# masa-ue/SVDD

Measured on AMD Instinct MI355X. Metric: decoded sequences/sec (whole node), L=200 M=10 128-step SVDD-MC, higher is better.
Workload: dtype f32; 1 GPU; DNA enhancer SVDD-MC, batch=256/GPU, L=200, M=10, 128 steps (BASELINE.json configs[1]); dilated-CNN backbone 3.3M params + ConvGRU value net; global_batch=256, rng=philox

## Files before the change

include/svdd_hip.h:

```cpp
#ifndef SVDD_HIP_H
#define SVDD_HIP_H

#include <stdint.h>

#ifdef __cplusplus
extern "C" {
#endif

#define SVDD_VOCAB 5
#define SVDD_MASK 4
#define SVDD_MAX_M 1024

enum {
  SVDD_OK = 0,
  SVDD_E_ARG = -1,
  SVDD_E_LAUNCH = -2,
  SVDD_E_NODEVICE = -3
};

enum {
  SVDD_LAYOUT_BLV = 0,
  SVDD_LAYOUT_BVL = 1
};

// ... 121 lines not shown

int svdd_transform_samples(const uint8_t* tok, int R, int L, int transposed, float* out,
                           void* stream);

int svdd_subs_logp(const float* logits, const uint8_t* x, int B, int L, int layout, float* logp,
                   void* stream);

int svdd_compact_flags(const int32_t* flags, int n, int32_t* live_idx, int32_t* slot, int32_t* count, void* stream);
int svdd_compact_by_key(const int32_t* key, int n, int32_t* live_idx, int32_t* slot, int32_t* count, int split, void* stream);
int svdd_gather_rows(const void* src, const int32_t* idx, const int32_t* count, int n, int row_bytes, void* dst, void* stream);
int svdd_advance_rows(const void* src, const int32_t* slot, const int32_t* sel, int B, int M, int row_bytes, void* dst,
                      void* stream);
int svdd_select_compact(const float* scores, const int32_t* slot, const float* parent_score, const uint8_t* cand, int B,
                        int L, int M, int mode, const svdd_rng_t* rng, uint8_t* x_next, float* soft, int32_t* idx,
                        float* sel_score, int32_t* changed, void* stream);

int svdd_tds_resample(const float* reward_num, const float* reward_den, double alpha,
                      const uint8_t* sample, const double* u, int B, int L,
                      uint8_t* x_next, int32_t* idx, double* work, void* stream);

int svdd_mt19937_uniform_f32(uint32_t* state, float* out, long long n, void* stream);

int svdd_gru_bidir_f32(const float* x, const float* wpack, const float* bpack, float* out, int n, int L,
                       const int32_t* count, void* stream);

int svdd_bb_layer_fwd_f32(const float* y, const float* bias, const float* f_prev, const float* tb, const float* gamma,
                          const float* beta, float eps, float* f_out, uint8_t* mask, float* hn, int64_t rows, int rows_per_seq,
                          int channels, void* stream);
int svdd_bb_layer_bwd_f32(const float* g_hn, const float* f_in, const float* tb, const float* gamma, float eps, const float* g_in,
                          const uint8_t* mask_prev, float* g_out, float* gt_out, int64_t rows, int rows_per_seq, int channels,
// ... 158 lines not shown
```

svdd_amd/_lib.py:

```python
import ctypes
import os
import subprocess

_HERE = os.path.dirname(os.path.abspath(__file__))
CSRC = os.path.join(_HERE, "csrc")
SO_PATH = os.environ.get("SVDD_HIP_LIB") or os.path.join(CSRC, "libsvdd_hip.so")
ABI_VERSION = 17

OK, E_ARG, E_LAUNCH, E_NODEVICE = 0, -1, -2, -3
LAYOUT_BLV, LAYOUT_BVL = 0, 1
RNG_REPLAY, RNG_PHILOX = 0, 1
SELECT_ARGMAX, SELECT_MULTINOMIAL = 0, 1
TARGET_MEAN, TARGET_LOGMEANEXP = 0, 1
EVOLVE_GLOBAL, EVOLVE_ROW = 0, 1
ATTR_GRADIENT, ATTR_TIMES_INPUT = 0, 1
PRECISIONS = {"f32": 0, "f16x3": 1, "bf16x3": 2, "f16": 3, "bf16": 4}
MAX_M = 1024
PATTERN_MAX_WIDTH = 32

OPT_FORCE_EXACT, OPT_MSPLIT, OPT_SELECT_ONE_ROW, OPT_BACKBONE_LP_VERSION, OPT_TRUNK_GEMM_VERSION = 0, 1, 2, 3, 4
OPT_CAND_ROW_STRIDE, OPT_TRUNK_PLANES_F32, OPT_BACKBONE_SPLIT, OPT_SELECT_BATCHES = 5, 6, 7, 8


class SvddRng(ctypes.Structure):
# ... 104 lines not shown
                         vp, vp, vp, vp, vp, vp, vp, vp, vp, vp, vp),
    "svdd_candidate_windows_tight": (vp, vp, i32, i32, i32, i32, vp, vp, vp),
    "svdd_kmer_counts": (vp, i32, i32, i32, vp, vp, vp),
    "svdd_pack_tokens": (vp, i32, i32, vp, vp, vp),
    "svdd_hamming_nn": (vp, vp, i32, i32, i32, i32, i32, i32, vp, vp, vp),
    "svdd_edit_nn": (vp, vp, i32, i32, i32, i32, i32, i32, i32, i32, vp, vp, vp),
    "svdd_within": (vp, vp, vp, vp, i32, i32, i32, i32, vp, vp, i32, vp),
    "svdd_greedy_pick": (vp, i32, vp, vp, i32, i32, i32, i32, vp, vp, vp, i32, vp, vp),
    "svdd_edit_within": (vp, vp, vp, i32, i32, i32, i32, i32, vp, vp, i32, vp),
    "svdd_edit_pairs": (vp, vp, vp, i32, i32, i32, i32, i32, i32, vp, vp),
    "svdd_motif_scan": (vp, i32, i32, vp, vp, vp, i32, i32, vp, vp, vp, vp, vp),
    "svdd_motif_reward": (vp, i32, i32, vp, vp, vp, vp, i32, i32, vp, vp, vp, vp, vp, f32, vp, vp, vp, vp),
    "svdd_candidate_parts": (vp, vp, i32, i32, i32, i32, i32, vp, vp, vp, vp, vp),
    "svdd_conv_tower_parts_f32": (vp, vp, vp, vp, vp, vp, i32, i32, i32, i32, i32, i32, vp, vp, vp),
    "svdd_backbone_incr4_f32": (vp, vp, vp, vp, vp, vp, i32, i32, i32, pi32, i32, vp, vp, vp, vp, i32, i32, vp, vp, i32, vp, i32, vp),
    "svdd_pattern_mutants": (vp, vp, vp, vp, vp, i32, i32, i32, i32, vp, vp, vp, vp),
    "svdd_pattern_fold": (vp, vp, vp, vp, i32, i32, i32, i32, i32, vp, vp, vp, vp, vp),
    "svdd_pattern_apply": (vp, vp, vp, vp, vp, vp, i32, i32, i32, i32, i32, vp, vp, vp, vp, vp, vp, vp, vp, vp, vp, vp, vp),
}
EXPORTS = tuple(SIGNATURES)


def build(force=False):
    import glob
    srcs = sorted(glob.glob(os.path.join(CSRC, "*.hip")) + glob.glob(os.path.join(CSRC, "*.h")) + [os.path.join(CSRC, "Makefile")])
    srcs.append(os.path.join(os.path.dirname(_HERE), "include", "svdd_hip.h"))
    if os.environ.get("SVDD_HIP_LIB"):
        return SO_PATH
    stale = not os.path.exists(SO_PATH) or os.path.getmtime(SO_PATH) < max(os.path.getmtime(f) for f in srcs)
    if force or stale:
# ... 123 lines not shown
```

svdd_amd/csrc/svdd_kernels.hip:

```cpp
#include <float.h>
#include <stdlib.h>
#include <string.h>

#include "svdd_host.h"

namespace {

constexpr int V = SVDD_VOCAB;
constexpr int MASK = SVDD_MASK;
constexpr float NEG_INF_F = -1000000.0f;
constexpr int WAVE = 64;

__device__ __forceinline__ float expf_cr(float x) { return (float)exp((double)x); }
__device__ __forceinline__ float logf_cr(float x) { return (float)log((double)x); }
__device__ __forceinline__ float expf_cr_small(float x) {
  const double d = (double)x;
  double p = 1.0 / 720.0;
  p = __builtin_fma(p, d, 1.0 / 120.0);
  p = __builtin_fma(p, d, 1.0 / 24.0);
  p = __builtin_fma(p, d, 1.0 / 6.0);
  p = __builtin_fma(p, d, 0.5);
  p = __builtin_fma(p, d, 1.0);
  p = __builtin_fma(p, d, 1.0);
  const long long low = __double_as_longlong(p) & 0x1FFFFFFFll;
// ... 1986 lines not shown
  const int b = blockIdx.x;
  const int sl = slot[(size_t)b * M + sel[b]];
  if (sl < 0) return;
  const uintptr_t al = (uintptr_t)row_bytes | reinterpret_cast<uintptr_t>(src) | reinterpret_cast<uintptr_t>(dst);
  if ((al & 15) == 0) {
    const uint4* s16 = reinterpret_cast<const uint4*>(src + (size_t)sl * row_bytes);
    uint4* d16 = reinterpret_cast<uint4*>(dst + (size_t)b * row_bytes);
    for (int i = threadIdx.x; i < (row_bytes >> 4); i += 256) d16[i] = s16[i];
  } else {
    const uint32_t* s4 = reinterpret_cast<const uint32_t*>(src + (size_t)sl * row_bytes);
    uint32_t* d4 = reinterpret_cast<uint32_t*>(dst + (size_t)b * row_bytes);
    for (int i = threadIdx.x; i < (row_bytes >> 2); i += 256) d4[i] = s4[i];
  }
}


constexpr int MT_N = 624, MT_M = 397, MT_GEN = MT_N - MT_M , MT_RING = 2048;

__device__ __forceinline__ uint32_t mt_tw(uint32_t a, uint32_t b) {
  const uint32_t y = (a & 0x80000000u) | (b & 0x7fffffffu);
  return (y >> 1) ^ ((b & 1u) ? 0x9908b0dfu : 0u);
}
__device__ __forceinline__ uint32_t mt_temper(uint32_t y) {
  y ^= (y >> 11);
  y ^= (y << 7) & 0x9d2c5680u;
  y ^= (y << 15) & 0xefc60000u;
  y ^= (y >> 18);
  return y;
}
__device__ __forceinline__ float mt_float(uint32_t x) { return (float)(mt_temper(x) & 0xFFFFFFu) * (1.0f / 16777216.0f); }
// ... 297 lines not shown

int svdd_gather_rows(const void* src, const int32_t* idx, const int32_t* count, int n, int row_bytes, void* dst, void* stream) {
  if (!src || !idx || !dst || n <= 0 || row_bytes <= 0) return SVDD_E_ARG;
  return svdd_launch(gather_rows_kernel, dim3((unsigned)((n + 3) / 4)), dim3(256), 0, stream, (const uint8_t*)src, idx, count, n,
                     row_bytes, (uint8_t*)dst);
}

int svdd_advance_rows(const void* src, const int32_t* slot, const int32_t* sel, int B, int M, int row_bytes, void* dst,
                      void* stream) {
  if (!src || !slot || !sel || !dst || B <= 0 || M <= 0 || row_bytes <= 0 || (row_bytes & 3)) return SVDD_E_ARG;
  if (((uintptr_t)src | (uintptr_t)dst) & 3) return SVDD_E_ARG;
  return svdd_launch(advance_rows_kernel, dim3((unsigned)B), dim3(256), 0, stream, (const uint8_t*)src, slot, sel, B, M, row_bytes,
                     (uint8_t*)dst);
}

static int launch_pos(void (*k)(PosArgs), const PosArgs& a, void* stream) {
  const int64_t N = (int64_t)a.R * a.L;
  return svdd_launch(k, dim3((unsigned)((N + 255) / 256)), dim3(256), 0, stream, a);
}

int svdd_x0hat(const float* logits, const uint8_t* xt, int R, int L, int layout, float* onehot_t, uint8_t* x0hat,
               void* stream) {
  if (!logits || !xt || (!onehot_t && !x0hat) || R <= 0 || L <= 0 || bad_layout(layout)) return SVDD_E_ARG;
  return launch_pos(x0hat_kernel, PosArgs{logits, xt, R, L, layout, onehot_t, x0hat, nullptr, 1}, stream);
}

int svdd_finalize(const float* logits, const uint8_t* x, int B, int L, int layout, int64_t* out_i64,
                  uint8_t* out_u8, void* stream) {
  if (!logits || !x || (!out_i64 && !out_u8) || B <= 0 || L <= 0 || bad_layout(layout)) return SVDD_E_ARG;
  return launch_pos(finalize_kernel, PosArgs{logits, x, B, L, layout, nullptr, out_u8, out_i64, 0}, stream);
// ... 291 lines not shown
```

svdd_amd/csrc/svdd_nets.hip:

```cpp
#include "svdd_host.h"
#include "svdd_device.h"

namespace {

constexpr int H = 64;
constexpr int HPAD = H + 4;

template <bool BOTH>
__global__ __launch_bounds__(BOTH ? 512 : 256) void gru_bidir_kernel(const float* __restrict__ x, const float* __restrict__ wpack,
                                                                     const float* __restrict__ bpack, float* __restrict__ out,
                                                                     int n_alloc, int L, int ts, const int* __restrict__ count) {
  __shared__ __attribute__((aligned(16))) float hbuf_all[BOTH ? 2 : 1][2][TS][HPAD];
  const int lane = threadIdx.x & 63;
  const int w = (threadIdx.x >> 6) & 3;
  const int dir = BOTH ? (int)(threadIdx.x >> 8) : (int)(blockIdx.x & 1);
  float (*hbuf)[TS][HPAD] = hbuf_all[BOTH ? dir : 0];
  const int j = lane & 15;
  const int g = lane >> 4;
  const int seq0 = (BOTH ? (int)blockIdx.x : (int)(blockIdx.x >> 1)) * ts;
  const int n = count ? __builtin_amdgcn_readfirstlane(*count) : n_alloc;
  if (seq0 >= n) return;

  float wr[96];
  {
// ... 1736 lines not shown
  for (int e = tid; e < tile_rows * 5; e += 512) {
    const int row = e / 5, v = e - 5 * row;
    const int q = SPT1 ? 0 : row % il, pos = SPT1 ? row : row / il;
    if (seq0 + q >= nvalid) continue;
    const float* hr = img + row * BB_AP;
    const float* wv = a.w2 + v * BB_C;
    float sm = a.w2[5 * BB_C + v];
#pragma unroll 8
    for (int k = 0; k < BB_C; ++k) sm += hr[k] * wv[k];
    const int64_t sq = (a.row_idx && a.out_scatter) ? (int64_t)a.row_idx[seq0 + q] : (int64_t)(seq0 + q);
    a.out[(sq * L + pos) * 5 + v] = sm;
  }
}
#undef BB_OWN

constexpr int SEG_SLOTS = 7;

struct BackboneSegArgs {
  const uint8_t* x;
  const float* table0;
  const float* tiles;
  const float* vec;
  float* planes;
  const int* items;
  int n, L, layer;
  const int* order;
  const int* order_count;
  int order_stride;
};

struct BackboneReach {
  int r[BB_MAXL];
// ... 158 lines not shown
        unsigned m = 0;
        if (rr < n)
          for (int e = 0; e < 8 && 8 * w8 + e < L; ++e) {
            const size_t at = (size_t)rr * L + 8 * w8 + e;
            const uint8_t a = x[at];
            if (keep) x_next[at] = a;
            m |= (unsigned)(a != x_cur[at]) << e;
          }
        chb[rl * 32 + w8] = (unsigned char)m;
      }
    }
    __syncthreads();
    const int r = r0 + tid;
    const u64 ch[4] = {chs[tid][0], chs[tid][1], chs[tid][2], chs[tid][3]};
    int* it = its[tid];
    int cnt = 0, nt = 0;
    if (tight) {
      int cend = -1, io = 0, il = 0;
#pragma unroll
      for (int q = 0; q < 4; ++q)
        for (u64 b = ch[q]; b; b &= b - 1) {
          const int p = 64 * q + __builtin_ctzll(b);
          const int lo = max(0, p - reach), hi = min(L - 1, p + reach);
          int o = lo > cend ? lo : cend + 1;
          for (; o <= hi; o += 16) {
            ++nt;
            if (il > 0 && il < max_item && o == io + 16 * il) { ++il; continue; }
            if (il > 0) { if (cnt < SEG_SLOTS) it[cnt] = io | il << 8; ++cnt; }
            io = o; il = 1;
          }
          cend = o - 1;
        }
      if (il > 0) { if (cnt < SEG_SLOTS) it[cnt] = io | il << 8; ++cnt; }
    }
    if (!tight || cnt > SEG_SLOTS) {
      int m = 0;
#pragma unroll
      for (int q = 0; q < 4; ++q)
        for (u64 b = ch[q]; b; b &= b - 1) {
          const int p = 64 * q + __builtin_ctzll(b);
          const int tlo = max(0, p - reach) >> 4, thi = min(L - 1, p + reach) >> 4;
          m |= ((2 << thi) - 1) & ~((1 << tlo) - 1);
        }
      cnt = 0; nt = __popc(m);
      for (int t = 0; t < TW_RT;) {
        if (!(m >> t & 1)) { ++t; continue; }
        int len = 1;
        while (len < max_item && t + len < TW_RT && (m >> (t + len) & 1)) ++len;
        it[cnt++] = (tight ? 16 * t : t) | len << 8;
        t += len;
      }
    }
    for (; cnt < SEG_SLOTS; ++cnt) it[cnt] = 0;
    tiles += nt;
#pragma unroll
    for (int s = 0; s < SEG_SLOTS; ++s) {
      item[s] = its[tid][s];
      if (r < n) itk[(size_t)r * SEG_SLOTS + s] = item[s];
#pragma unroll
      for (int c = 0; c < 4; ++c) cnt4[c] += (item[s] >> 8) == 4 - c;
    }
    __syncthreads();
  }
  if (stat) {
#pragma unroll
    for (int off = 32; off > 0; off >>= 1) tiles += __shfl_xor(tiles, off, 64);
    if (lane == 0 && tiles) atomicAdd(stat + (tight ? 0 : 1), (unsigned long long)tiles);
  }
// ... 909 lines not shown
static size_t seg_lds_bytes(int rows, bool pad) {
  size_t bytes = sizeof(float) * ((size_t)rows * BB_AP + 5 * (size_t)rows + rows + 8);
  if (pad && g_incr_residency > 0) {
    const size_t least = (CU_LDS_BYTES / (size_t)(g_incr_residency + 1) / 1024 + 1) * 1024;
    if (least > bytes) bytes = least;
  }
  return bytes;
}

enum IncrList { INCR_SLOT, INCR_ORDERED, INCR_TIGHT };

struct IncrCall {
  const uint8_t* x; const float *table0, *tiles, *vec, *w2; float* out; int n, L, nlayers; const int* dilations; int lead;
  float* planes; uint8_t* x_prev; int32_t* items; unsigned long long* stat; int first, max_item;
  int32_t *order, *order_count; int depth; uint8_t* x_prev2; int parity; void* stream;
};

typedef void (*BackboneSegKernel)(BackboneSegArgs);
static BackboneSegKernel backbone_seg_choice(IncrList list, int mi, bool dilation4) {
  if (dilation4) return mi == 4 ? backbone_seg_kernel<4, true, 4> : mi == 2 ? backbone_seg_kernel<2, true, 4> : backbone_seg_kernel<1, true, 4>;
  if (list == INCR_TIGHT) return backbone_seg_tight_kernel;
  if (list == INCR_SLOT) return mi == 4 ? backbone_seg_kernel<4> : backbone_seg_kernel<2>;
  return mi == 4 ? backbone_seg_kernel<4, true> : mi == 2 ? backbone_seg_kernel<2, true> : backbone_seg_kernel<1, true>;
}

static int backbone_incr(IncrList list, const IncrCall& c) {
  const bool ordered = list != INCR_SLOT, tight = list == INCR_TIGHT;
  const int n = c.n, L = c.L, mi = c.max_item, lead = c.lead, depth = c.depth;
  if (!c.x || !c.table0 || !c.tiles || !c.vec || !c.w2 || !c.out || !c.dilations || !c.planes || !c.x_prev || !c.items || n <= 0 ||
      L <= TW_ROWS / 2 || L > TW_ROWS || c.nlayers <= 0 || c.nlayers > BB_MAXL || lead < 2 || lead > c.nlayers || depth < lead ||
      depth > c.nlayers || !(mi == 2 || (mi == 4 && !tight) || (mi == 1 && list == INCR_ORDERED)) ||
      (ordered && (!c.order || !c.order_count || n > 65536)) ||
      (tight && (!c.x_prev2 || c.x_prev2 == c.x_prev || (c.parity != 0 && c.parity != 1))))
    return SVDD_E_ARG;
  for (int i = 0; i < depth; ++i) if (c.dilations[i] != (i < lead ? 1 : 4)) return SVDD_E_ARG;
  BackboneArgs a;
  if (!backbone_args(a, c.x, c.table0, c.tiles, c.vec, c.w2, c.out, n, L, 1, c.nlayers, c.dilations)) return SVDD_E_ARG;
  a.planes = c.planes; a.planes_P = depth;
  uint8_t* x_cur = c.parity ? c.x_prev2 : c.x_prev;
  uint8_t* x_next = c.parity ? c.x_prev : c.x_prev2;
  const SvddLds lds = svdd_lds_raised(backbone_lds_bytes(c.nlayers, 3));
  SvddSpan span(SVDD_SLOT_BACKBONE);
  if (c.first) {
    if (hipMemcpyAsync(x_cur, c.x, (size_t)n * L, hipMemcpyDeviceToDevice, (hipStream_t)c.stream) != hipSuccess) return SVDD_E_LAUNCH;
    return svdd_launch_timed(span.all(), backbone_kernel<true, false, 1>, dim3((unsigned)n), dim3(512), lds, c.stream, a, BackboneSave{});
  }
  const int slots = mi == 1 ? TW_RT : SEG_SLOTS;
  const BackboneReach reach = backbone_reach(c.dilations, depth, lead);
  int rc;
  if (tight) {
    rc = svdd_launch_timed(span.first(), backbone_list_kernel, dim3((unsigned)depth), dim3(256), 0, c.stream, c.x, (const uint8_t*)x_cur, x_next,
                           n, L, mi, c.items, c.order, c.order_count, c.stat, reach);
  } else {
    rc = svdd_launch_timed(span.first(), mi == 1 ? backbone_worklist_kernel<TW_RT> : backbone_worklist_kernel<SEG_SLOTS>,
                           dim3((unsigned)((n + 3) / 4)), dim3(256), 0, c.stream, c.x, c.x_prev, n, L, depth, mi, c.items, c.stat, reach);
    if (rc == SVDD_OK && ordered)
      rc = svdd_launch(mi == 1 ? backbone_order_kernel<TW_RT> : backbone_order_kernel<SEG_SLOTS>, dim3((unsigned)depth), dim3(256), 0, c.stream,
                       c.items, n, c.order, c.order_count);
  }
  if (rc != SVDD_OK) return SVDD_E_LAUNCH;
  BackboneSegArgs sa{c.x, c.table0, c.tiles, c.vec, c.planes, c.items, n, L, 0, nullptr, nullptr, 0};
  if (ordered) { sa.order = c.order; sa.order_count = c.order_count; sa.order_stride = n * slots; }
  const BackboneSegKernel seg[2] = {backbone_seg_choice(list, mi, false), backbone_seg_choice(list, mi, true)};
  const size_t slds[2] = {seg_lds_bytes(tight ? 16 * mi + 8 : 16 * (mi + 2), ordered), seg_lds_bytes(16 * (mi + 2), ordered)};
  svdd_raise_lds_limit(seg[0], slds[0]);
  if (depth > lead) svdd_raise_lds_limit(seg[1], slds[1]);
  const dim3 sgrid((unsigned)n * slots);
  for (int k = 1; k <= depth; ++k) {
    sa.layer = k;
    if (svdd_launch(seg[k > lead], sgrid, dim3(256), slds[k > lead], c.stream, sa) != SVDD_OK) return SVDD_E_LAUNCH;
  }
  return svdd_launch_timed(span.last(), backbone_kernel<true, false, 2>, dim3((unsigned)n), dim3(512), lds, c.stream, a, BackboneSave{});
}

extern "C" int svdd_backbone_incr_f32(const uint8_t* x, const float* table0, const float* tiles, const float* vec, const float* w2,
                                      float* out, int n, int L, int nlayers, const int* dilations, int lead, float* planes,
                                      uint8_t* x_prev, int32_t* items, unsigned long long* stat, int first, int max_item,
                                      void* stream) {
  return backbone_incr(INCR_SLOT, IncrCall{x, table0, tiles, vec, w2, out, n, L, nlayers, dilations, lead, planes, x_prev, items, stat, first,
                                           max_item, nullptr, nullptr, lead, nullptr, 0, stream});
}

extern "C" int svdd_backbone_incr2_f32(const uint8_t* x, const float* table0, const float* tiles, const float* vec, const float* w2,
                                       float* out, int n, int L, int nlayers, const int* dilations, int lead, float* planes,
                                       uint8_t* x_prev, int32_t* items, unsigned long long* stat, int first, int max_item,
// ... 5 lines not shown
extern "C" int svdd_backbone_incr3_f32(const uint8_t* x, const float* table0, const float* tiles, const float* vec, const float* w2,
                                       float* out, int n, int L, int nlayers, const int* dilations, int lead, float* planes,
                                       uint8_t* x_prev, int32_t* items, unsigned long long* stat, int first, int max_item,
                                       int32_t* order, int32_t* order_count, int depth, void* stream) {
  return backbone_incr(INCR_ORDERED, IncrCall{x, table0, tiles, vec, w2, out, n, L, nlayers, dilations, lead, planes, x_prev, items, stat, first,
                                              max_item, order, order_count, depth, nullptr, 0, stream});
}

extern "C" int svdd_backbone_incr4_f32(const uint8_t* x, const float* table0, const float* tiles, const float* vec, const float* w2,
                                       float* out, int n, int L, int nlayers, const int* dilations, int lead, float* planes,
                                       uint8_t* x_prev, int32_t* items, unsigned long long* stat, int first, int max_item,
                                       int32_t* order, int32_t* order_count, int depth, uint8_t* x_prev2, int parity,
                                       void* on_stream) {
  return backbone_incr(INCR_TIGHT, IncrCall{x, table0, tiles, vec, w2, out, n, L, nlayers, dilations, lead, planes, x_prev, items, stat, first,
                                            max_item, order, order_count, depth, x_prev2, parity, on_stream});
}

typedef decltype(&value_tail_kernel<1>) ValueTailKernel;

extern "C" int svdd_value_tail_f32(const float* h_fwd, const float* h_bwd, const float* w1pack, const float* b1,
                                   const float* w_eff, const float* b_eff, float* out, int n, int L, int n_tasks,
                                   const int32_t* count, void* stream) {
  if (!h_fwd || !h_bwd || !w1pack || !b1 || !w_eff || !b_eff || !out || n <= 0 || L <= 0 || n_tasks < 1 || n_tasks > 4)
    return SVDD_E_ARG;
  ValueTailKernel kern;
  switch (n_tasks) {
    case 1: kern = value_tail_kernel<1>; break;
    case 2: kern = value_tail_kernel<2>; break;
    case 3: kern = value_tail_kernel<3>; break;
    default: kern = value_tail_kernel<4>; break;
// ... 56 lines not shown
```

svdd_amd/diffusion.py:

```python
import contextlib
import functools
import math
import os
import warnings
import weakref
from dataclasses import dataclass
from typing import Optional

import numpy as np
import torch
import torch.nn.functional as F
from torch import nn

from . import noise_schedule, ops
from .backbone import CNNModel


@dataclass
class Loss:
    loss: torch.Tensor
    nlls: torch.Tensor
    token_mask: torch.Tensor


# ... 158 lines not shown
        self.row_offset = 0
        self._shard = None
        self.fuse_nets = True
        self.precision = "f32"
        self.skip_unchanged = True
        self.late_steps_from = "auto"
        self.dedup_prior = True
        self.dps_fused = True
        self.dps_one_launch = True
        self._dps_hard_onehot, self._dps_raw_logits, self._dps_logp = False, None, None
        self.dps_single_forward = False
        self.logits_cache = "auto"
        self.incremental_backbone = "auto"
        self.incremental_depth = os.environ.get("SVDD_INCR_DEPTH") or "auto"
        self.incremental_items = os.environ.get("SVDD_INCR_ITEMS") or "tight"
        self.skip_stats = None
        self.skip_generic = False
        self.trace = None
        self.state_trace = None
        self._sched_cache = {}
        self._fused = WeightCache()
        self._scope_depth, self._scope_id = 0, 0
        self.fuse_trunk_f32 = True
        self.replay_rng = "device"
        self._replay_stream = None
        self._replay_checked = None
        self._classifier_fused_last = None
        self.elbo_trace = None
        self._from_state = False
        self.cdq_draws = 10
# ... 1437 lines not shown
            self.count = self.count3[0:1]
            self.row_idx, self.row_slot = torch.empty(B, **i32), torch.empty(B, **i32)
            self.row_count = torch.zeros(1, **i32)
            self.parent_score, self.sel_score = torch.empty(B, device=dev), torch.empty(B, device=dev)
            self.changed, self.idx = torch.empty(B, **i32), torch.empty(B, **i32)
            self.parent_out, self.parent_out_lp, self.seq = None, None, None
            self.M = M
            self.n_live = torch.zeros(1, dtype=torch.int64, device=dev)
            self.n_changed = torch.zeros(1, dtype=torch.int64, device=dev)
            self.late = False
            self.split_bufs = None
            self.prior_rows_identical = False
            self.n_win_rows = None
            self.n_tile_layers = None

    def _select_compact(self, sc, ws, cand, step):
        mode, rng = self._select_args(step)
        x_next, _, _, _ = ops.select_compact(sc, ws.slot, ws.parent_score, cand, mode=mode, rng=rng, sel_score=ws.sel_score,
                                             changed=ws.changed, idx=ws.idx)
        ws.parent_score, ws.sel_score = ws.sel_score, ws.parent_score
        if ws.parent_out is not None and ws.seq is not None:
            ops.advance_rows(ws.seq, ws.slot, ws.idx, ws.parent_out, ws.M)
        if self.skip_stats is not None:
            ws.n_live += ws.count
            ws.n_changed += ws.changed.sum()
        return x_next

    def _dense_scores(self, sc, ws, B, M):
        live = ws.slot >= 0
        return torch.where(live, sc[ws.slot.clamp(min=0).long()], ws.parent_score.repeat_interleave(M)).view(B, M)

    def _finish_stats(self, ws, B, M, S, kind):
        if self.skip_stats is not None:
            self.skip_stats.update(kind=kind, steps=S, candidates=B * M * S, live_candidates=int(ws.n_live),
                                   row_steps=B * S, changed_row_steps=int(ws.n_changed),
                                   tower_window_rows=None if ws.n_win_rows is None else int(round(float(ws.n_win_rows))),
                                   tower_tile_layers=None if ws.n_tile_layers is None else int(ws.n_tile_layers))
# ... 34 lines not shown
            ws.n_win_rows = torch.zeros(1, dtype=torch.float64, device=self.device)
            ws.n_tile_layers = torch.zeros(1, dtype=torch.int64, device=self.device)
        from .fused import FusedValueNet
        dedup = self._prior_dedup_ok(x) and isinstance(fn, FusedValueNet)
        ws.parent_score.copy_(fn.forward_tokens(x[:1].contiguous()).reshape(1).expand(B) if dedup
                              else fn.forward_tokens(x).reshape(B))
        ws.prior_rows_identical = dedup
        fb = self._fused_backbone_or_none(L) if self._use_logits_cache(L) else None
        share = hasattr(fn, "candidates_ok") and fn.candidates_ok(L, M)
        toks_c = None if share else torch.empty((B * M, L), dtype=torch.uint8, device=self.device)
        logits = None
        inc, stem = (None, None) if fb is not None else self._incremental_stem(B, L)
        if stem is not None:
            stem.stat.zero_()
            stem.forwards = 0
        auto_late = share and self.late_steps_from == "auto" and not _capturing() and hasattr(fn, "gru_round_rows")
        if auto_late:
            live_host = torch.empty(1, dtype=torch.int32).pin_memory()
            live_ev, live_pending, live_last = torch.cuda.Event(), False, 0
            late_thr = 0.97 * fn.gru_round_rows()
        for i in range(S):
            if inc is not None:
                logits = inc.forward_incremental(x, stem, out=logits)
            elif fb is None or logits is None:
                logits = self._prior_logits(x) if i == 0 else self._backbone_logits(x)
            else:
                ops.compact_flags(ws.changed, ws.row_idx, ws.row_slot, ws.row_count)
                fb.forward_rows(x, count=ws.row_count, out=logits, row_idx=ws.row_idx, scatter=True)
            ops.propose(logits, x, sched[i, 2], sched[i, 1], M, self._rng(i, M, B, L, logits), cand=cand, onehot=onehot)
            if share:
# ... 7 lines not shown
                sc = fn.candidate_scores_compact(onehot, cand, x, ws).reshape(-1)
                if auto_late and not live_pending:
                    live_host.copy_(ws.count, non_blocking=True)
                    live_ev.record()
                    live_pending = True
            else:
                candidate_windows(cand, x, margin=0, flags=ws.flags)
                ops.compact_flags(ws.flags, ws.live_idx, ws.slot, ws.count)
                ops.gather_rows(cand.view(B * M, L), ws.live_idx, ws.count, toks_c)
                if getattr(fn, "share_level0", False):
                    sc = fn.forward_tokens(toks_c, count=ws.count, shared=(x, ws.live_idx, M)).reshape(-1)
                else:
                    sc = fn.forward_tokens(toks_c, count=ws.count).reshape(-1)
            if self.trace is not None or self.state_trace is not None:
                self._record(logits, self._dense_scores(sc, ws, B, M), x)
            x = self._select_compact(sc, ws, cand, i)
        self._finish_stats(ws, B, M, S, "mc")
        if inc is None:
            return self._noise_removal(x)
        if self.config.sampling.noise_removal:
            logits = inc.forward_incremental(x, stem, out=logits)
        if self.skip_stats is not None:
            marked = stem.stat.tolist()
            self.skip_stats.update(backbone_stem_tile_layers=marked[0],
                                   backbone_stem_tile_layers_dense=stem.forwards * B * ((L + 15) // 16) * stem.lead,
                                   backbone_deep_tile_layers=marked[1],
                                   backbone_deep_tile_layers_dense=stem.forwards * B * ((L + 15) // 16) * stem.deep)
        return self._noise_removal(x, logits=logits)

    def _controlled_sample_generic_skipping(self, fn, x, cand, onehot, sched, B, L, S, M):
        from .fused import candidate_windows
# ... 239 lines not shown
```

svdd_amd/fused.py:

```python
import ctypes
import os
import math

import torch
import torch.nn.functional as F
from torch import nn

from . import _lib
from .backbone import CNNModel
from .value_nets import ConvGRUTrunk, ConvHead


def _cl(w):
    return w.detach().unsqueeze(2).contiguous(memory_format=torch.channels_last)


def pack_gru(gru):
    H = gru.hidden_size
    assert H == 64 and gru.input_size == 64 and gru.bidirectional and gru.num_layers == 1 and gru.bias
    packs, biases = [], []
    for sfx in ("", "_reverse"):
        w_ih = getattr(gru, "weight_ih_l0" + sfx).detach().float()
        w_hh = getattr(gru, "weight_hh_l0" + sfx).detach().float()
        b_ih = getattr(gru, "bias_ih_l0" + sfx).detach().float()
# ... 338 lines not shown


class IncrementalStem:

    def __init__(self, n, L, lead, dev, deep=0, tight=False):
        self.n, self.L, self.lead, self.deep, self.tight = n, L, lead, deep, tight
        depth = lead + deep
        self.planes = torch.empty((depth, n, 208, 128), dtype=torch.float32, device=dev)
        self.x_prev = torch.empty((n, L), dtype=torch.uint8, device=dev)
        self.x_prev2 = torch.empty((n, L), dtype=torch.uint8, device=dev)
        self.parity = 0
        self.items = torch.zeros((depth, n, INCR_SLOTS), dtype=torch.int32, device=dev)
        self.order = torch.zeros((depth, n * INCR_SLOTS), dtype=torch.int32, device=dev)
        self.order_count = torch.zeros(depth, dtype=torch.int32, device=dev)
        self.stat = torch.zeros(2, dtype=torch.int64, device=dev)
        self.valid = False
        self.forwards = 0


def backbone_cnn_incremental(tokens, pk, st, out=None, max_item=None):
    assert tokens.is_cuda and tokens.dtype == torch.uint8 and tokens.is_contiguous() and tuple(tokens.shape) == (st.n, st.L)
    n, L = tokens.shape
    if out is None:
        out = torch.empty((n, L, 5), dtype=torch.float32, device=tokens.device)
    dil = (ctypes.c_int * len(pk["dil"]))(*pk["dil"])
    first = not st.valid
    max_item = int(max_item or INCR_MAX_ITEM)
    tight = st.tight and max_item == 2
    if tight:
        entry, extra = "svdd_backbone_incr4_f32", (st.order, st.order_count, st.lead + st.deep, st.x_prev2, st.parity)
    elif st.deep > 0:
        entry, extra = "svdd_backbone_incr3_f32", (st.order, st.order_count, st.lead + st.deep)
    elif INCR_ORDERED:
        entry, extra = "svdd_backbone_incr2_f32", (st.order, st.order_count)
    else:
        entry, extra = "svdd_backbone_incr_f32", ()
    stream = ctypes.c_void_p(torch.cuda.current_stream().cuda_stream)
    _lib.call(entry, tokens, pk["table0"], pk["tiles"], pk["vec"], pk["w2"], out, n, L, len(pk["dil"]), dil, st.lead, st.planes, st.x_prev,
              st.items, st.stat, int(first), max_item, *extra, stream)
    if tight and not first:
        st.parity ^= 1
    st.valid = True
    st.forwards += 0 if first else 1
# ... 606 lines not shown

    def incremental_ok(self, n, L, any_batch=False):
        return (self.kernel_ok(L) and self.precision == "f32" and 104 < L <= 208 and leading_dilation1(self.ol_dil) >= 2 and
                (any_batch or (n > BB_SPLIT_MAX_SEQ and not 0 < n % 256 <= BB_SPLIT_MAX_SEQ)))

    def incremental_stem(self, n, L, depth=None, tight=False):
        lead = leading_dilation1(self.ol_dil)
        deep = 0 if depth is None else int(depth) - lead
        if not 0 <= deep <= following_dilation4(self.ol_dil):
            raise ValueError(f"incremental depth {depth}: expected {lead} .. {lead + following_dilation4(self.ol_dil)}")
        key = (n, L, deep, self.ol_tiles.device)
        st = self._incr.get(key)
        if st is None:
            self._incr.clear()
            st = self._incr[key] = IncrementalStem(n, L, lead, self.ol_tiles.device, deep)
        st.valid, st.tight = False, bool(tight)
        return st

    def forward_incremental(self, tok, st, out=None):
        return backbone_cnn_incremental(tok, self.ol_pack(), st, out)

    def _lp_pack(self):
        pk = self._lp.get(self.precision)
        if pk is None:
            pk = self._lp[self.precision] = pack_backbone_lp(self._cnn[0], self.precision)
        return pk

    def forward_rows(self, tok, count=None, out=None, row_idx=None, scatter=False):
        if self.precision != "f32":
            return backbone_cnn_lp(tok, self._lp_pack(), count, out, row_idx, scatter)
        return backbone_cnn(tok, self.ol_pack(), count, out, row_idx, scatter)
# ... 41 lines not shown
```

svdd_amd/ops.py:

```python
import ctypes
from dataclasses import dataclass
from typing import Optional

import torch

from . import _lib
from ._lib import (LAYOUT_BLV, LAYOUT_BVL, RNG_PHILOX, RNG_REPLAY, SELECT_ARGMAX,
                   SELECT_MULTINOMIAL, SvddError, SvddRng)

MASK = 4


@dataclass
class Rng:
    uniforms: Optional[torch.Tensor] = None
    seed: int = 0
    row_offset: int = 0
    step: int = 0
    uniforms_layout: Optional[int] = None
    uniforms_rows: int = 0

    def c_struct(self, logits_layout=LAYOUT_BLV):
        if self.uniforms is not None:
            ul = logits_layout if self.uniforms_layout is None else self.uniforms_layout
# ... 854 lines not shown

def gather_rows(src, idx, count, dst):
    n = src.shape[0]
    row_bytes = src[0].numel() * src.element_size()
    _lib.call("svdd_gather_rows", src, idx, count, n, row_bytes, dst)
    return dst


def advance_rows(src, slot, sel, dst, M):
    B = dst.shape[0]
    row_bytes = dst[0].numel() * dst.element_size()
    _lib.call("svdd_advance_rows", src, slot, sel, B, M, row_bytes, dst)
    return dst


def x0hat(logits, xt, want_tokens=False, want_onehot=True):
    logits = _need(logits, torch.float32, "logits")
    xt = _need(xt, torch.uint8, "xt").contiguous()
    R, L = xt.shape
    logits, layout = layout_of(logits)
    oh = torch.empty((R, 4, L), dtype=torch.float32, device=xt.device) if want_onehot else None
    xh = torch.empty((R, L), dtype=torch.uint8, device=xt.device) if want_tokens else None
    _lib.call("svdd_x0hat", logits, xt, R, L, layout, oh, xh)
    return oh, xh


def finalize(logits, x):
    logits = _need(logits, torch.float32, "logits")
    x = _need(x, torch.uint8, "x").contiguous()
    B, L = x.shape
# ... 205 lines not shown
```

Measured before the change: 812.9 sequences/s.

## Fuse selection, row advance and incremental work-list build into one kernel

```diff
diff --git a/include/svdd_hip.h b/include/svdd_hip.h
--- a/include/svdd_hip.h
+++ b/include/svdd_hip.h
@@ -159,6 +159,15 @@
 int svdd_select_compact(const float* scores, const int32_t* slot, const float* parent_score, const uint8_t* cand, int B,
                         int L, int M, int mode, const svdd_rng_t* rng, uint8_t* x_next, float* soft, int32_t* idx,
                         float* sel_score, int32_t* changed, void* stream);
+int svdd_select_advance_list(const float* scores, const int32_t* slot, const float* parent_score, const uint8_t* cand, int B, int L,
+                             int M, int mode, const svdd_rng_t* rng, uint8_t* x_next, int32_t* idx, float* sel_score,
+                             int32_t* changed, const void* adv_src, void* adv_dst, int row_bytes, const uint8_t* x_cur,
+                             uint8_t* x_keep, int lead, int depth, int max_item, int32_t* items, int32_t* order,
+                             int32_t* order_count, unsigned long long* stat, int32_t* ticket, void* on_stream);
+int svdd_backbone_incr4_listed_f32(const uint8_t* x, const float* table0, const float* tiles, const float* vec, const float* w2,
+                                   float* out, int n, int L, int nlayers, const int* dilations, int lead, float* planes,
+                                   uint8_t* x_prev, int32_t* items, unsigned long long* stat, int max_item, int32_t* order,
+                                   int32_t* order_count, int depth, uint8_t* x_prev2, int parity, void* on_stream);
 
 int svdd_tds_resample(const float* reward_num, const float* reward_den, double alpha,
                       const uint8_t* sample, const double* u, int B, int L,
diff --git a/svdd_amd/_lib.py b/svdd_amd/_lib.py
--- a/svdd_amd/_lib.py
+++ b/svdd_amd/_lib.py
@@ -142,6 +142,9 @@
     "svdd_candidate_parts": (vp, vp, i32, i32, i32, i32, i32, vp, vp, vp, vp, vp),
     "svdd_conv_tower_parts_f32": (vp, vp, vp, vp, vp, vp, i32, i32, i32, i32, i32, i32, vp, vp, vp),
     "svdd_backbone_incr4_f32": (vp, vp, vp, vp, vp, vp, i32, i32, i32, pi32, i32, vp, vp, vp, vp, i32, i32, vp, vp, i32, vp, i32, vp),
+    "svdd_select_advance_list": (vp, vp, vp, vp, i32, i32, i32, i32, RNG, vp, vp, vp, vp, vp, vp, i32, vp, vp, i32, i32, i32, vp, vp, vp, vp, vp,
+                                 vp),
+    "svdd_backbone_incr4_listed_f32": (vp, vp, vp, vp, vp, vp, i32, i32, i32, pi32, i32, vp, vp, vp, vp, i32, vp, vp, i32, vp, i32, vp),
     "svdd_pattern_mutants": (vp, vp, vp, vp, vp, i32, i32, i32, i32, vp, vp, vp, vp),
     "svdd_pattern_fold": (vp, vp, vp, vp, i32, i32, i32, i32, i32, vp, vp, vp, vp, vp),
     "svdd_pattern_apply": (vp, vp, vp, vp, vp, vp, i32, i32, i32, i32, i32, vp, vp, vp, vp, vp, vp, vp, vp, vp, vp, vp, vp),
diff --git a/svdd_amd/csrc/svdd_cut_body.h b/svdd_amd/csrc/svdd_cut_body.h
--- /dev/null
+++ b/svdd_amd/csrc/svdd_cut_body.h
@@ -0,0 +1,38 @@
+  int cnt = 0, nt = 0;
+  if (tight) {
+    int cend = -1, io = 0, il = 0;
+#pragma unroll
+    for (int q = 0; q < 4; ++q)
+      for (u64 b = ch[q]; b; b &= b - 1) {
+        const int p = 64 * q + __builtin_ctzll(b);
+        const int lo = max(0, p - reach), hi = min(L - 1, p + reach);
+        int o = lo > cend ? lo : cend + 1;
+        for (; o <= hi; o += 16) {
+          ++nt;
+          if (il > 0 && il < max_item && o == io + 16 * il) { ++il; continue; }
+          if (il > 0) { if (cnt < SEG_SLOTS) it[cnt] = io | il << 8; ++cnt; }
+          io = o; il = 1;
+        }
+        cend = o - 1;
+      }
+    if (il > 0) { if (cnt < SEG_SLOTS) it[cnt] = io | il << 8; ++cnt; }
+  }
+  if (!tight || cnt > SEG_SLOTS) {
+    int m = 0;
+#pragma unroll
+    for (int q = 0; q < 4; ++q)
+      for (u64 b = ch[q]; b; b &= b - 1) {
+        const int p = 64 * q + __builtin_ctzll(b);
+        const int tlo = max(0, p - reach) >> 4, thi = min(L - 1, p + reach) >> 4;
+        m |= ((2 << thi) - 1) & ~((1 << tlo) - 1);
+      }
+    cnt = 0; nt = __popc(m);
+    for (int t = 0; t < TW_RT;) {
+      if (!(m >> t & 1)) { ++t; continue; }
+      int len = 1;
+      while (len < max_item && t + len < TW_RT && (m >> (t + len) & 1)) ++len;
+      it[cnt++] = (tight ? 16 * t : t) | len << 8;
+      t += len;
+    }
+  }
+  for (; cnt < SEG_SLOTS; ++cnt) it[cnt] = 0;
diff --git a/svdd_amd/csrc/svdd_items.h b/svdd_amd/csrc/svdd_items.h
--- /dev/null
+++ b/svdd_amd/csrc/svdd_items.h
@@ -0,0 +1,9 @@
+#pragma once
+
+#include "svdd_host.h"
+
+constexpr int SEG_SLOTS = 7;
+
+__host__ __device__ inline int backbone_reach_of(int k, int lead1) {
+  return 4 + 4 * (k < lead1 ? k : lead1) + 16 * (k > lead1 ? k - lead1 : 0);
+}
diff --git a/svdd_amd/csrc/svdd_kernels.hip b/svdd_amd/csrc/svdd_kernels.hip
--- a/svdd_amd/csrc/svdd_kernels.hip
+++ b/svdd_amd/csrc/svdd_kernels.hip
@@ -3,6 +3,7 @@
 #include <string.h>
 
 #include "svdd_host.h"
+#include "svdd_items.h"
 
 namespace {
 
@@ -2024,6 +2025,143 @@
   }
 }
 
+struct StepListArgs {
+  const uint8_t* adv_src; uint8_t* adv_dst; int row_bytes;
+  const uint8_t* x_cur; uint8_t* x_keep;
+  int lead1, depth, max_item;
+  int32_t *items, *order, *order_count; unsigned long long* stat; int32_t* ticket;
+};
+
+template <int MP, int MS>
+__global__ __launch_bounds__(1024) void select_advance_list_kernel(SelectArgs a, StepListArgs s) {
+  typedef unsigned long long u64;
+  __shared__ u64 chs[4];
+  __shared__ int its[BB_MAXL][SEG_SLOTS];
+  __shared__ int sh_best, sh_last;
+  const int tid = threadIdx.x, lane = tid & (WAVE - 1), wave = tid >> 6;
+  const int row = blockIdx.x, n = gridDim.x;
+  if (wave == 0) {
+    SelectArgs one = a;
+    one.B = row + 1;
+    const int wb = select_decide<MP, 1, MS>(one, row, lane);
+    if (lane == 0) sh_best = wb;
+  }
+  __syncthreads();
+  const int best = sh_best;
+  if (wave < 4) {
+    bool diff = false;
+    if (tid < a.L) {
+      const uint8_t w = a.cand[((int64_t)row * a.M + best) * a.ld + tid], c = s.x_cur[(size_t)row * a.L + tid];
+      a.x_next[(size_t)row * a.L + tid] = w;
+      s.x_keep[(size_t)row * a.L + tid] = w;
+      diff = w != c;
+    }
+    const u64 m = __ballot(diff);
+    if (lane == 0) chs[wave] = m;
+  }
+  __syncthreads();
+  if (tid < s.depth) {
+    const u64 ch[4] = {chs[0], chs[1], chs[2], chs[3]};
+    const int L = a.L, reach = backbone_reach_of(tid + 1, s.lead1), max_item = s.max_item;
+    const bool tight = tid < s.lead1;
+    int* it = its[tid];
+#include "svdd_cut_body.h"
+    int32_t* out = s.items + ((size_t)tid * n + row) * SEG_SLOTS;
+#pragma unroll
+    for (int q = 0; q < SEG_SLOTS; ++q) __hip_atomic_store(out + q, it[q], __ATOMIC_RELAXED, __HIP_MEMORY_SCOPE_AGENT);
+    (void)nt;
+  }
+  asm volatile("s_waitcnt vmcnt(0)" ::: "memory");
+  __syncthreads();
+  if (tid == 0) {
+    __threadfence();
+    asm volatile("s_waitcnt vmcnt(0)" ::: "memory");
+    const int last = atomicAdd(s.ticket, 1) == n - 1;
+    if (last) {
+      __threadfence();
+      asm volatile("s_waitcnt vmcnt(0)" ::: "memory");
+    }
+    sh_last = last;
+  }
+  if (s.adv_src) {
+    const int sl = a.slot[(int64_t)row * a.M + best];
+    if (sl >= 0) {
+      const uintptr_t al = (uintptr_t)s.row_bytes | reinterpret_cast<uintptr_t>(s.adv_src) | reinterpret_cast<uintptr_t>(s.adv_dst);
+      if ((al & 15) == 0) {
+        const uint4* s16 = reinterpret_cast<const uint4*>(s.adv_src + (size_t)sl * s.row_bytes);
+        uint4* d16 = reinterpret_cast<uint4*>(s.adv_dst + (size_t)row * s.row_bytes);
+        for (int i = tid; i < (s.row_bytes >> 4); i += 1024) d16[i] = s16[i];
+      } else {
+        const uint32_t* s4 = reinterpret_cast<const uint32_t*>(s.adv_src + (size_t)sl * s.row_bytes);
+        uint32_t* d4 = reinterpret_cast<uint32_t*>(s.adv_dst + (size_t)row * s.row_bytes);
+        for (int i = tid; i < (s.row_bytes >> 2); i += 1024) d4[i] = s4[i];
+      }
+    }
+  }
+  __syncthreads();
+  if (!sh_last) return;
+  for (int k = wave; k < s.depth; k += 16) {
+    const int32_t* itk = s.items + (size_t)k * n * SEG_SLOTS;
+    int32_t* ord = s.order + (size_t)k * n * SEG_SLOTS;
+    int item[4][SEG_SLOTS], tot[4] = {0, 0, 0, 0}, tiles = 0;
+    for (int r0 = 0; r0 < n; r0 += 256) {
+#pragma unroll
+      for (int q = 0; q < 4; ++q) {
+        const int r = r0 + 64 * q + lane;
+#pragma unroll
+        for (int e = 0; e < SEG_SLOTS; ++e)
+          item[q][e] = r < n ? __hip_atomic_load(itk + (size_t)r * SEG_SLOTS + e, __ATOMIC_RELAXED, __HIP_MEMORY_SCOPE_AGENT) : 0;
+      }
+#pragma unroll
+      for (int q = 0; q < 4; ++q)
+#pragma unroll
+        for (int e = 0; e < SEG_SLOTS; ++e) {
+          tiles += item[q][e] >> 8;
+#pragma unroll
+          for (int c = 0; c < 4; ++c) tot[c] += (item[q][e] >> 8) == 4 - c;
+        }
+    }
+#pragma unroll
+    for (int off = 32; off > 0; off >>= 1) {
+      tiles += __shfl_xor(tiles, off, WAVE);
+#pragma unroll
+      for (int c = 0; c < 4; ++c) tot[c] += __shfl_xor(tot[c], off, WAVE);
+    }
+    int base[4], run = 0;
+#pragma unroll
+    for (int c = 0; c < 4; ++c) { base[c] = run; run += tot[c]; }
+    if (lane == 0) {
+      s.order_count[k] = run;
+      if (s.stat && tiles) atomicAdd(s.stat + (k < s.lead1 ? 0 : 1), (u64)tiles);
+    }
+    for (int r0 = 0; r0 < n; r0 += 256) {
+#pragma unroll
+      for (int q = 0; q < 4; ++q) {
+        const int r = r0 + 64 * q + lane;
+        int cl[4] = {0, 0, 0, 0};
+#pragma unroll
+        for (int e = 0; e < SEG_SLOTS; ++e) {
+          if (n > 256) item[q][e] = r < n ? __hip_atomic_load(itk + (size_t)r * SEG_SLOTS + e, __ATOMIC_RELAXED, __HIP_MEMORY_SCOPE_AGENT) : 0;
+#pragma unroll
+          for (int c = 0; c < 4; ++c) cl[c] += (item[q][e] >> 8) == 4 - c;
+        }
+#pragma unroll
+        for (int c = 0; c < 4; ++c) {
+          int v = cl[c];
+#pragma unroll
+          for (int off = 1; off < 64; off <<= 1) { const int u = __shfl_up(v, off, WAVE); if (lane >= off) v += u; }
+          int at = base[c] + v - cl[c];
+#pragma unroll
+          for (int e = 0; e < SEG_SLOTS; ++e)
+            if ((item[q][e] >> 8) == 4 - c) ord[at++] = r << 16 | item[q][e];
+          base[c] += __shfl(v, 63, WAVE);
+        }
+      }
+    }
+  }
+  if (tid == 0) __hip_atomic_store(s.ticket, 0, __ATOMIC_RELAXED, __HIP_MEMORY_SCOPE_AGENT);
+}
+
 
 constexpr int MT_N = 624, MT_M = 397, MT_GEN = MT_N - MT_M , MT_RING = 2048;
 
@@ -2351,6 +2489,41 @@
                      (uint8_t*)dst);
 }
 
+int svdd_select_advance_list(const float* scores, const int32_t* slot, const float* parent_score, const uint8_t* cand, int B, int L,
+                             int M, int mode, const svdd_rng_t* rng, uint8_t* x_next, int32_t* idx, float* sel_score,
+                             int32_t* changed, const void* adv_src, void* adv_dst, int row_bytes, const uint8_t* x_cur,
+                             uint8_t* x_keep, int lead, int depth, int max_item, int32_t* items, int32_t* order,
+                             int32_t* order_count, unsigned long long* stat, int32_t* ticket, void* on_stream) {
+  if (!scores || !slot || !parent_score || !cand || !x_next || !idx || !x_cur || !x_keep || !items || !order || !order_count || !ticket ||
+      B <= 0 || B > 65536 || L <= TW_ROWS / 2 || L > TW_ROWS || M <= 0 || M > WAVE || lead < 2 || depth < lead || depth > BB_MAXL ||
+      max_item != 2 || x_keep == x_cur || x_next == x_cur || x_next == x_keep)
+    return SVDD_E_ARG;
+  if (mode != SVDD_SELECT_ARGMAX && mode != SVDD_SELECT_MULTINOMIAL) return SVDD_E_ARG;
+  if (mode == SVDD_SELECT_MULTINOMIAL && (!rng || rng->kind != SVDD_RNG_PHILOX)) return SVDD_E_ARG;
+  if (!adv_src != !adv_dst) return SVDD_E_ARG;
+  if (adv_src && (row_bytes <= 0 || (row_bytes & 3) || (((uintptr_t)adv_src | (uintptr_t)adv_dst) & 3))) return SVDD_E_ARG;
+  SelectArgs a{scores, cand, B, L, M, mode, rng ? rng->step : 0u, rng ? rng->seed : 0ull, rng ? rng->row_offset : 0ull, x_next, nullptr,
+               idx, slot, parent_score, sel_score, changed, g_cand_ld >= L ? g_cand_ld : L};
+  const StepListArgs s{(const uint8_t*)adv_src, (uint8_t*)adv_dst, row_bytes, x_cur, x_keep, lead, depth, max_item, items, order, order_count,
+                       stat, ticket};
+  int mp = 1;
+  while (mp < M) mp <<= 1;
+  void (*kern)(SelectArgs, StepListArgs);
+  if (M == 10) kern = select_advance_list_kernel<16, 10>;
+  else if (M == 20) kern = select_advance_list_kernel<32, 20>;
+  else switch (mp) {
+    case 1: kern = select_advance_list_kernel<1, 1>; break;
+    case 2: kern = select_advance_list_kernel<2, 2>; break;
+    case 4: kern = select_advance_list_kernel<4, 4>; break;
+    case 8: kern = select_advance_list_kernel<8, 8>; break;
+    case 16: kern = select_advance_list_kernel<16, 16>; break;
+    case 32: kern = select_advance_list_kernel<32, 32>; break;
+    default: kern = select_advance_list_kernel<64, 64>; break;
+  }
+  SvddSpan span(SVDD_SLOT_SELECT);
+  return svdd_launch_timed(span.all(), kern, dim3((unsigned)B), dim3(1024), 0, on_stream, a, s);
+}
+
 static int launch_pos(void (*k)(PosArgs), const PosArgs& a, void* stream) {
   const int64_t N = (int64_t)a.R * a.L;
   return svdd_launch(k, dim3((unsigned)((N + 255) / 256)), dim3(256), 0, stream, a);
diff --git a/svdd_amd/csrc/svdd_nets.hip b/svdd_amd/csrc/svdd_nets.hip
--- a/svdd_amd/csrc/svdd_nets.hip
+++ b/svdd_amd/csrc/svdd_nets.hip
@@ -1,5 +1,6 @@
 #include "svdd_host.h"
 #include "svdd_device.h"
+#include "svdd_items.h"
 
 namespace {
 
@@ -1774,8 +1775,6 @@
 }
 #undef BB_OWN
 
-constexpr int SEG_SLOTS = 7;
-
 struct BackboneSegArgs {
   const uint8_t* x;
   const float* table0;
@@ -1964,44 +1963,7 @@
     const int r = r0 + tid;
     const u64 ch[4] = {chs[tid][0], chs[tid][1], chs[tid][2], chs[tid][3]};
     int* it = its[tid];
-    int cnt = 0, nt = 0;
-    if (tight) {
-      int cend = -1, io = 0, il = 0;
-#pragma unroll
-      for (int q = 0; q < 4; ++q)
-        for (u64 b = ch[q]; b; b &= b - 1) {
-          const int p = 64 * q + __builtin_ctzll(b);
-          const int lo = max(0, p - reach), hi = min(L - 1, p + reach);
-          int o = lo > cend ? lo : cend + 1;
-          for (; o <= hi; o += 16) {
-            ++nt;
-            if (il > 0 && il < max_item && o == io + 16 * il) { ++il; continue; }
-            if (il > 0) { if (cnt < SEG_SLOTS) it[cnt] = io | il << 8; ++cnt; }
-            io = o; il = 1;
-          }
-          cend = o - 1;
-        }
-      if (il > 0) { if (cnt < SEG_SLOTS) it[cnt] = io | il << 8; ++cnt; }
-    }
-    if (!tight || cnt > SEG_SLOTS) {
-      int m = 0;
-#pragma unroll
-      for (int q = 0; q < 4; ++q)
-        for (u64 b = ch[q]; b; b &= b - 1) {
-          const int p = 64 * q + __builtin_ctzll(b);
-          const int tlo = max(0, p - reach) >> 4, thi = min(L - 1, p + reach) >> 4;
-          m |= ((2 << thi) - 1) & ~((1 << tlo) - 1);
-        }
-      cnt = 0; nt = __popc(m);
-      for (int t = 0; t < TW_RT;) {
-        if (!(m >> t & 1)) { ++t; continue; }
-        int len = 1;
-        while (len < max_item && t + len < TW_RT && (m >> (t + len) & 1)) ++len;
-        it[cnt++] = (tight ? 16 * t : t) | len << 8;
-        t += len;
-      }
-    }
-    for (; cnt < SEG_SLOTS; ++cnt) it[cnt] = 0;
+#include "svdd_cut_body.h"
     tiles += nt;
 #pragma unroll
     for (int s = 0; s < SEG_SLOTS; ++s) {
@@ -2941,6 +2903,7 @@
   const uint8_t* x; const float *table0, *tiles, *vec, *w2; float* out; int n, L, nlayers; const int* dilations; int lead;
   float* planes; uint8_t* x_prev; int32_t* items; unsigned long long* stat; int first, max_item;
   int32_t *order, *order_count; int depth; uint8_t* x_prev2; int parity; void* stream;
+  int ready;
 };
 
 typedef void (*BackboneSegKernel)(BackboneSegArgs);
@@ -2958,7 +2921,7 @@
       L <= TW_ROWS / 2 || L > TW_ROWS || c.nlayers <= 0 || c.nlayers > BB_MAXL || lead < 2 || lead > c.nlayers || depth < lead ||
       depth > c.nlayers || !(mi == 2 || (mi == 4 && !tight) || (mi == 1 && list == INCR_ORDERED)) ||
       (ordered && (!c.order || !c.order_count || n > 65536)) ||
-      (tight && (!c.x_prev2 || c.x_prev2 == c.x_prev || (c.parity != 0 && c.parity != 1))))
+      (tight && (!c.x_prev2 || c.x_prev2 == c.x_prev || (c.parity != 0 && c.parity != 1))) || (c.ready && (!tight || c.first)))
     return SVDD_E_ARG;
   for (int i = 0; i < depth; ++i) if (c.dilations[i] != (i < lead ? 1 : 4)) return SVDD_E_ARG;
   BackboneArgs a;
@@ -2974,8 +2937,9 @@
   }
   const int slots = mi == 1 ? TW_RT : SEG_SLOTS;
   const BackboneReach reach = backbone_reach(c.dilations, depth, lead);
-  int rc;
-  if (tight) {
+  int rc = SVDD_OK;
+  if (c.ready) {
+  } else if (tight) {
     rc = svdd_launch_timed(span.first(), backbone_list_kernel, dim3((unsigned)depth), dim3(256), 0, c.stream, c.x, (const uint8_t*)x_cur, x_next,
                            n, L, mi, c.items, c.order, c.order_count, c.stat, reach);
   } else {
@@ -2995,7 +2959,9 @@
   const dim3 sgrid((unsigned)n * slots);
   for (int k = 1; k <= depth; ++k) {
     sa.layer = k;
-    if (svdd_launch(seg[k > lead], sgrid, dim3(256), slds[k > lead], c.stream, sa) != SVDD_OK) return SVDD_E_LAUNCH;
+    rc = c.ready && k == 1 ? svdd_launch_timed(span.first(), seg[0], sgrid, dim3(256), slds[0], c.stream, sa)
+                           : svdd_launch(seg[k > lead], sgrid, dim3(256), slds[k > lead], c.stream, sa);
+    if (rc != SVDD_OK) return SVDD_E_LAUNCH;
   }
   return svdd_launch_timed(span.last(), backbone_kernel<true, false, 2>, dim3((unsigned)n), dim3(512), lds, c.stream, a, BackboneSave{});
 }
@@ -3031,6 +2997,14 @@
                                        void* on_stream) {
   return backbone_incr(INCR_TIGHT, IncrCall{x, table0, tiles, vec, w2, out, n, L, nlayers, dilations, lead, planes, x_prev, items, stat, first,
                                             max_item, order, order_count, depth, x_prev2, parity, on_stream});
+}
+
+extern "C" int svdd_backbone_incr4_listed_f32(const uint8_t* x, const float* table0, const float* tiles, const float* vec, const float* w2,
+                                              float* out, int n, int L, int nlayers, const int* dilations, int lead, float* planes,
+                                              uint8_t* x_prev, int32_t* items, unsigned long long* stat, int max_item, int32_t* order,
+                                              int32_t* order_count, int depth, uint8_t* x_prev2, int parity, void* on_stream) {
+  return backbone_incr(INCR_TIGHT, IncrCall{x, table0, tiles, vec, w2, out, n, L, nlayers, dilations, lead, planes, x_prev, items, stat, 0,
+                                            max_item, order, order_count, depth, x_prev2, parity, on_stream, 1});
 }
 
 typedef decltype(&value_tail_kernel<1>) ValueTailKernel;
diff --git a/svdd_amd/diffusion.py b/svdd_amd/diffusion.py
--- a/svdd_amd/diffusion.py
+++ b/svdd_amd/diffusion.py
@@ -196,6 +196,7 @@
         self.incremental_backbone = "auto"
         self.incremental_depth = os.environ.get("SVDD_INCR_DEPTH") or "auto"
         self.incremental_items = os.environ.get("SVDD_INCR_ITEMS") or "tight"
+        self.step_chain = os.environ.get("SVDD_STEP_CHAIN") or "fused"
         self.skip_stats = None
         self.skip_generic = False
         self.trace = None
@@ -1663,13 +1664,19 @@
             self.n_win_rows = None
             self.n_tile_layers = None
 
-    def _select_compact(self, sc, ws, cand, step):
+    def _select_compact(self, sc, ws, cand, step, stem=None):
         mode, rng = self._select_args(step)
-        x_next, _, _, _ = ops.select_compact(sc, ws.slot, ws.parent_score, cand, mode=mode, rng=rng, sel_score=ws.sel_score,
-                                             changed=ws.changed, idx=ws.idx)
+        advance = ws.parent_out is not None and ws.seq is not None
+        if stem is not None:
+            x_next, _, _, _ = ops.select_advance_list(sc, ws.slot, ws.parent_score, cand, stem, mode=mode, rng=rng, sel_score=ws.sel_score,
+                                                      changed=ws.changed, idx=ws.idx, adv_src=ws.seq if advance else None,
+                                                      adv_dst=ws.parent_out if advance else None)
+        else:
+            x_next, _, _, _ = ops.select_compact(sc, ws.slot, ws.parent_score, cand, mode=mode, rng=rng, sel_score=ws.sel_score,
+                                                 changed=ws.changed, idx=ws.idx)
+            if advance:
+                ops.advance_rows(ws.seq, ws.slot, ws.idx, ws.parent_out, ws.M)
         ws.parent_score, ws.sel_score = ws.sel_score, ws.parent_score
-        if ws.parent_out is not None and ws.seq is not None:
-            ops.advance_rows(ws.seq, ws.slot, ws.idx, ws.parent_out, ws.M)
         if self.skip_stats is not None:
             ws.n_live += ws.count
             ws.n_changed += ws.changed.sum()
@@ -1734,6 +1741,12 @@
         if stem is not None:
             stem.stat.zero_()
             stem.forwards = 0
+        if self.step_chain not in ("fused", "split"):
+            raise ValueError(f"step_chain = {self.step_chain!r}: expected 'fused' or 'split'")
+        from .fused import INCR_MAX_ITEM
+        chain = (self.step_chain == "fused" and stem is not None and stem.tight and INCR_MAX_ITEM == 2 and self.rng_mode == "philox" and
+                 M <= 64 and self.trace is None and self.state_trace is None)
+        more = self.config.sampling.noise_removal
         auto_late = share and self.late_steps_from == "auto" and not _capturing() and hasattr(fn, "gru_round_rows")
         if auto_late:
             live_host = torch.empty(1, dtype=torch.int32).pin_memory()
@@ -1771,7 +1784,7 @@
                     sc = fn.forward_tokens(toks_c, count=ws.count).reshape(-1)
             if self.trace is not None or self.state_trace is not None:
                 self._record(logits, self._dense_scores(sc, ws, B, M), x)
-            x = self._select_compact(sc, ws, cand, i)
+            x = self._select_compact(sc, ws, cand, i, stem if chain and (i + 1 < S or more) else None)
         self._finish_stats(ws, B, M, S, "mc")
         if inc is None:
             return self._noise_removal(x)
diff --git a/svdd_amd/fused.py b/svdd_amd/fused.py
--- a/svdd_amd/fused.py
+++ b/svdd_amd/fused.py
@@ -376,6 +376,8 @@
         self.order = torch.zeros((depth, n * INCR_SLOTS), dtype=torch.int32, device=dev)
         self.order_count = torch.zeros(depth, dtype=torch.int32, device=dev)
         self.stat = torch.zeros(2, dtype=torch.int64, device=dev)
+        self.ticket = torch.zeros(1, dtype=torch.int32, device=dev)
+        self.listed = False
         self.valid = False
         self.forwards = 0
 
@@ -389,6 +391,14 @@
     first = not st.valid
     max_item = int(max_item or INCR_MAX_ITEM)
     tight = st.tight and max_item == 2
+    listed, st.listed = st.listed, False
+    if listed:
+        assert tight and not first
+        _lib.call("svdd_backbone_incr4_listed_f32", tokens, pk["table0"], pk["tiles"], pk["vec"], pk["w2"], out, n, L, len(pk["dil"]), dil,
+                  st.lead, st.planes, st.x_prev, st.items, st.stat, max_item, st.order, st.order_count, st.lead + st.deep, st.x_prev2,
+                  st.parity, ctypes.c_void_p(torch.cuda.current_stream().cuda_stream))
+        st.forwards += 1
+        return out
     if tight:
         entry, extra = "svdd_backbone_incr4_f32", (st.order, st.order_count, st.lead + st.deep, st.x_prev2, st.parity)
     elif st.deep > 0:
@@ -1025,7 +1035,7 @@
         if st is None:
             self._incr.clear()
             st = self._incr[key] = IncrementalStem(n, L, lead, self.ol_tiles.device, deep)
-        st.valid, st.tight = False, bool(tight)
+        st.valid, st.tight, st.listed = False, bool(tight), False
         return st
 
     def forward_incremental(self, tok, st, out=None):
diff --git a/svdd_amd/ops.py b/svdd_amd/ops.py
--- a/svdd_amd/ops.py
+++ b/svdd_amd/ops.py
@@ -892,6 +892,29 @@
     return dst
 
 
+def select_advance_list(scores_c, slot, parent_score, cand, stem, mode=SELECT_ARGMAX, rng=None, x_next=None, sel_score=None, changed=None,
+                        idx=None, adv_src=None, adv_dst=None, max_item=2):
+    cand = _need(cand, torch.uint8, "cand").contiguous()
+    B, M, L = cand.shape
+    dev = cand.device
+    assert stem.tight and stem.valid and not stem.listed and (stem.n, stem.L) == (B, L), "the stem's planes must belong to this batch"
+    scores_c = _need(scores_c, torch.float32, "scores").contiguous()
+    x_next = torch.empty((B, L), dtype=torch.uint8, device=dev) if x_next is None else x_next
+    idx = torch.empty((B,), dtype=torch.int32, device=dev) if idx is None else idx
+    sel_score = torch.empty((B,), dtype=torch.float32, device=dev) if sel_score is None else sel_score
+    changed = torch.empty((B,), dtype=torch.int32, device=dev) if changed is None else changed
+    row_bytes = 0 if adv_dst is None else adv_dst[0].numel() * adv_dst.element_size()
+    rs = rng.c_struct() if rng is not None else None
+    x_cur, x_keep = (stem.x_prev2, stem.x_prev) if stem.parity else (stem.x_prev, stem.x_prev2)
+    stream = ctypes.c_void_p(torch.cuda.current_stream().cuda_stream)
+    _lib.call("svdd_select_advance_list", scores_c, slot, parent_score, cand, B, L, M, mode, ctypes.byref(rs) if rs is not None else None,
+              x_next, idx, sel_score, changed, adv_src, adv_dst, row_bytes, x_cur, x_keep, stem.lead, stem.lead + stem.deep, int(max_item),
+              stem.items, stem.order, stem.order_count, stem.stat, stem.ticket, stream)
+    stem.parity ^= 1
+    stem.listed = True
+    return x_next, idx, sel_score, changed
+
+
 def x0hat(logits, xt, want_tokens=False, want_onehot=True):
     logits = _need(logits, torch.float32, "logits")
     xt = _need(xt, torch.uint8, "xt").contiguous()
```

After: 810.2 sequences/s. About the same (-0.3%).
